# bxh1/VIDO-SLAM

Hardware: AMD Instinct MI355X
Metric: frames/sec end-to-end (flow+depth+track+local-BA) at 640x480; BA iters/sec (higher is better)
Workload: dtype f32

## Files before the change

include/vido_c.h:

```cpp
#ifndef VIDO_C_H
#define VIDO_C_H
#include <stdint.h>
#include <stddef.h>
#ifdef __cplusplus
extern "C" {
#endif

#define VIDO_OK              0
#define VIDO_E_INVALID      -1
#define VIDO_E_NO_DEVICE    -2
#define VIDO_E_HIP          -3
#define VIDO_E_CAPACITY     -4
#define VIDO_E_NOMEM        -5

#define VIDO_MAX_LEVELS 16

typedef struct vido_ctx vido_ctx;

typedef struct vido_keypoint { float x, y, size, angle, response; int32_t octave; } vido_keypoint;

typedef struct vido_config {
    int32_t device;
    int32_t width, height;
    int32_t max_batch;
// ... 159 lines not shown

typedef struct vido_ba_dynamic {
    int32_t n_H, n_dyn, n_tern, n_smooth;
    double* H_T;
    double* dyn_xyz;
    const int32_t* dyn_cam; const double* dyn_meas;
    const int32_t* tern_prev; const int32_t* tern_cur; const int32_t* tern_H;
    const int32_t* sm_i; const int32_t* sm_j;
    double info_dyn, info_tern, info_smooth, huber_dyn, huber_tern, huber_smooth;
} vido_ba_dynamic;
int vido_ba_optimize_dynamic(vido_ctx* ctx, vido_ba_problem* prob, vido_ba_dynamic* dyn, vido_ba_result* result,
                             vido_allreduce_fn allreduce, void* user);

int vido_correlation(vido_ctx* ctx, const float* first, const float* second, int B, int C, int H, int W, int stride,
                     float* out, int on_device);
int vido_det_order(vido_ctx* ctx, const float* scores, const long long* labels, const int* n_det, float confidence, int cap, long long* order, long long* labels_out, long long* n_live);
int vido_det_order_n(vido_ctx* ctx, const float* scores, const long long* labels, const int* n_det, float confidence, int cap, long long* order, long long* labels_out, long long* n_live,
                     int32_t* n_live32);
int vido_roi_levels(vido_ctx* ctx, const float* boxes, int n, float k_min, float k_max, int* out);
int vido_mask_logit_select(vido_ctx* ctx, const float* feat, const float* w, const float* b, const long long* labels, float* out, int n, int c, int hw, int classes);
int vido_mask_logit_select_n(vido_ctx* ctx, const float* feat, const float* w, const float* b, const long long* labels, float* out, int n, int c, int hw, int classes, const int32_t* n_live);
int vido_bias_act(vido_ctx* ctx, float* x, const float* bias, int N, int C, int H, int W, float slope);
int vido_bias_unary(vido_ctx* ctx, float* x, const float* bias, int N, int C, int H, int W, int kind);
int vido_upcat_reflect(vido_ctx* ctx, const float* x, const float* skip, int C1, int C2, int h, int w, float* out);
int vido_minmax_norm_u16(vido_ctx* ctx, const float* d, const float* mm, int64_t n, int32_t* out);
int vido_bias_res_act(vido_ctx* ctx, float* x, const float* bias, const float* res, int N, int C, int H, int W, float slope);
int vido_area_feed(vido_ctx* ctx, const uint8_t* bgr, int H, int W, float* out, int OH, int OW, float div);
int vido_backwarp(vido_ctx* ctx, const float* x, const float* flow, int B, int C, int H, int W, float* out);
int vido_deconv4s2_depthwise(vido_ctx* ctx, const float* x, const float* weight, int B, int C, int H, int W, float input_slope, float* out);

int vido_conv1x1_supported(int cin, int cout, int hw);
int vido_conv1x1_layout(int cin, int cout, int hw);
int vido_conv1x1_set_arith(int arith);
int vido_conv1x1_range_flag(vido_ctx* ctx, int reset);
int vido_range_latch(vido_ctx* ctx, unsigned* dst);
int vido_conv1x1_bias_act(vido_ctx* ctx, const float* x, const float* w_packed, const float* bias, const float* residual, float* y, int cin, int cout, int hw, float slope);
int vido_deconv2x2_supported(int n, int cin, int cout, int h, int w);
int vido_deconv2x2_bias_act(vido_ctx* ctx, const float* x, const float* w_packed, const float* bias, float* y, int n, int cin, int cout, int h, int w, float slope);
int vido_deconv2x2_bias_act_n(vido_ctx* ctx, const float* x, const float* w_packed, const float* bias, float* y, int n, int cin, int cout, int h, int w, float slope, const int32_t* n_live);
int vido_conv1x1_bias_up2_act(vido_ctx* ctx, const float* x, const float* w_packed, const float* bias, const float* residual_half, float* y, int cin, int cout, int h, int w, float slope);

int vido_conv_kxk_c2(vido_ctx* ctx, const float* x, const float* w, const float* bias, const float* residual, float* y, int cin, int k, int h, int w_);
int vido_conv1x1_skinny(vido_ctx* ctx, const float* x, const float* w_packed, const float* bias, const float* residual, float* y, int cin, int cout, long long hw, float slope);
int vido_stem7x7s2_pool(vido_ctx* ctx, const float* x, const float* w_packed, const float* bias, float* y, int h, int w);

int vido_conv_direct_supported(int cin, int cout, int h, int w, int kh, int kw, int sh, int sw, int ph, int pw);
long long vido_conv_direct_packed_floats(int cin, int cout, int kh, int kw);
int vido_conv_direct_pack(const float* w, int cin, int cout, int kh, int kw, float* w_packed);
int vido_conv_direct_bias_act(vido_ctx* ctx, const float* x, const float* w_packed, const float* bias, float* y, int n, int cin, int cout, int h, int w,
                              int kh, int kw, int sh, int sw, int ph, int pw, float slope);

int vido_wino3x3_supported(int cin, int cout, int h, int w);
int vido_wino3x3_fills_chip(int n, int cout, int h, int w, int min_wgs);
long long vido_wino3x3_packed_floats(int cin, int cout);
int vido_wino3x3_pack(const float* w, int cin, int cout, float* u_packed);
int vido_wino3x3_bias_act(vido_ctx* ctx, const float* x, const float* u_packed, const float* bias, float* y, int n, int cin, int cout, int h, int w, float slope);
int vido_wino3x3_form(int n, int cin, int cout, int h, int w);
int vido_fc_h_splitk(int rows, int k, int outs);
int vido_fc_h(vido_ctx* ctx, const float* x, const void* w_packed, const float* bias, float* part, float* y, int rows, int k, int outs, float slope);
int vido_conv3x3_h_supported(int n, int cin, int cout, int h, int w);
int vido_conv3x3_h_workgroups(int n, int cout, int h, int w);
int vido_conv3x3_h_bias_act(vido_ctx* ctx, const float* x, const void* w_packed, const float* bias, float* y, int n, int cin, int cout, int h, int w, float slope);
int vido_conv3x3_h_bias_act_n(vido_ctx* ctx, const float* x, const void* w_packed, const float* bias, float* y, int n, int cin, int cout, int h, int w, float slope, const int32_t* n_live);
int vido_conv3x3_h_live_form(int n, int cout, int h, int w, int live, int* channels, int* block_rows);
int vido_mask_head_coarse(void);
int vido_conv3x3_h_bias_act_form(vido_ctx* ctx, const float* x, const void* w_packed, const float* bias, float* y, int n, int cin, int cout, int h, int w, float slope, int rpw, int cg);
long long vido_wino3x3_packed_floats_form(int cin, int cout, int form);
int vido_wino3x3_pack_form(const float* w, int cin, int cout, int form, float* u_packed);
int vido_wino3x3_bias_act_form(vido_ctx* ctx, const float* x, const float* u_packed, const float* bias, float* y, int n, int cin, int cout, int h, int w, float slope, int form);
int vido_gconv3x3_supported(int H, int W, int cpg_in, int cpg_out);
int64_t vido_gconv3x3_packed_size(int groups, int cpg_in, int cpg_out);
int vido_gconv3x3_bias_act(vido_ctx* ctx, const float* x, const float* in_bias, const float* w_packed, const float* bias, float* y, int groups, int cpg_in, int cpg_out, int H, int W, float slope);
int vido_gconv3x3_s2_supported(int H, int W, int cpg_in, int cpg_out);
int vido_gconv3x3_s2_bias_act(vido_ctx* ctx, const float* x, const float* w_packed, const float* bias, float* y, int groups, int cpg_in, int cpg_out, int H, int W, float slope);
int vido_lfn_reg_front(vido_ctx* ctx, const float* im1, const float* im2, const float* flow, const float* mean, float scale, int B, int C, int H, int W, float* out, int out_channels);
int vido_lfn_reg_tail(vido_ctx* ctx, const float* dist, const float* flow, const float* wx, const float* bx, const float* wy, const float* by, int B, int K, int H, int W, float* out);
int vido_roi_align(vido_ctx* ctx, const float* feat, int B, int C, int H, int W, const float* rois, int n_rois,
                   float spatial_scale, int pooled_h, int pooled_w, int sampling_ratio, float* out, int on_device);
int vido_nms(vido_ctx* ctx, const float* boxes_xyxy, const float* scores, int n, float thresh, int32_t* keep_out,
             int32_t* n_keep, int on_device);
int vido_nms_grouped(vido_ctx* ctx, const float* boxes_xyxy, const float* scores, const int32_t* groups, int n, float thresh,
                     int32_t* keep_out, int32_t* n_keep, int on_device);
int vido_nms_segments(vido_ctx* ctx, const float* boxes_xyxy, const int32_t* groups, const int32_t* seg_off, const int32_t* seg_n, int n_seg, int max_n, int total,
                      float thresh, int32_t* keep_out, int32_t* n_keep);
int vido_roi_align_fpn(vido_ctx* ctx, const float* const feat[4], const int H[4], const int W[4], const float scale[4], int C, const float* boxes, const int32_t* level,
                       int n, int pooled_h, int pooled_w, int sampling_ratio, float* out);
int vido_nchw_to_nhwc(vido_ctx* ctx, const float* src, int B, int C, int H, int W, float* dst);
int vido_roi_align_fpn_nhwc(vido_ctx* ctx, const float* const feat[4], const int H[4], const int W[4], const float scale[4], int C, const float* boxes, const int32_t* level,
                            int n, int pooled_h, int pooled_w, int sampling_ratio, float* out);
int vido_roi_align_fpn_nhwc_n(vido_ctx* ctx, const float* const feat[4], const int H[4], const int W[4], const float scale[4], int C, const float* boxes, const int32_t* level,
                              int n, int pooled_h, int pooled_w, int sampling_ratio, float* out, const int32_t* n_live);
int vido_bawin_create(vido_ctx* ctx, int cap_frames, int cap_features);
int vido_bawin_push_frame(vido_ctx* ctx, int frame, int n, const double* meas, const float* xyz, const int32_t* asso);
int vido_bawin_set_labels(vido_ctx* ctx, int n, const int32_t* quads);
int vido_bawin_solve(vido_ctx* ctx, int start, int N, vido_ba_problem* prob, vido_ba_result* res, int32_t* n_obs_out, int32_t* n_pt_out);
int vido_bawin_read_points(vido_ctx* ctx, int frame, int n, float* xyz_out);
int vido_rpn_select(vido_ctx* ctx, int n_levels, const float* const* logits, const float* const* deltas, const int* h, const int* w, const int* stride, const float* cell_anchors,
                    int A, int K, int img_w, int img_h, float* boxes_out, float* scores_out, int32_t* n_out);
int vido_rpn_merge(vido_ctx* ctx, const float* boxes, const float* scores, const int32_t* keep, const int32_t* cnt, int n_levels, int K, int post_nms_top_n, int n_final,
                   float* out_boxes, float* out_scores, int32_t* n_valid);
int vido_det_class_sort(vido_ctx* ctx, const float* prob, const float* deltas, const float* proposals, const float* objectness, int N, int nc, float thresh, const float weights[4],
                        int img_w, int img_h, float* seg_boxes, int32_t* order, int32_t* seg_n);
int vido_det_select(vido_ctx* ctx, const float* prob, const float* seg_boxes, const int32_t* order, const int32_t* keep, const int32_t* cnt, int N, int nc, int detections_per_img, int cap,
                    int32_t* scratch, float* out_boxes, float* out_scores, int64_t* out_labels, int32_t* n_det);
int vido_mask_label_image(vido_ctx* ctx, const float* masks, const float* boxes, const int64_t* labels, int n, int M, int padding, float thresh, int H, int W, uint8_t* out);
// ... 81 lines not shown
```

vido-slam_amd/csrc/conv1x1.hip:

```cpp
#include "common.hpp"
#include <atomic>

namespace {
typedef float f32x16 __attribute__((ext_vector_type(16)));
typedef float f32x4 __attribute__((ext_vector_type(4)));
typedef float f32x2 __attribute__((ext_vector_type(2)));

#define C1_TM 128
#define C1_TN 128

struct C1Args { const float* x; const float* wp; const float* bias; const float* res; float* y; int M, N, K, mt, total, nchunk; float slope; unsigned xbytes, wbytes; int W; unsigned* range_flag; int hwimg, c4; const int* n_live; };

template <int RES, int KC>
__global__ __launch_bounds__(256) void k_conv1x1(C1Args A)
{
    constexpr int NG = KC / 8;
    constexpr int A_BUF = 4 * NG * 256, B_BUF = KC * C1_TN;
    constexpr int NPW = KC / 4;
    extern __shared__ __attribute__((aligned(16))) float c1_lds[];
    float* Al = c1_lds; float* Bl = c1_lds + 2 * A_BUF;
    const int tid = threadIdx.x, lane = tid & 63, w = __builtin_amdgcn_readfirstlane(tid >> 6), wm = w & 1, wn = w >> 1;
    const int per = gridDim.x >> 3, item = (blockIdx.x & 7) * per + (blockIdx.x >> 3);
    if (item >= A.total) return;
    const int nt = item / A.mt, mtile = item - nt * A.mt, n0 = nt * C1_TN, m0 = mtile * C1_TM;
// ... 413 lines not shown
    } else {
        float* X = (float*)L;
        if (g == 0) { ep_load(0, E0); ep_load(1, E1); } else { ep_load(2, E0); ep_load(3, E1); }
        __builtin_amdgcn_s_barrier();
        auto put = [&](int which, const f32x16& v0, const f32x16& v1) {
            float* Pw = X + (((which * 4 + w) * 2) * 16) * 64 + lane;
#pragma unroll
            for (int r = 0; r < 16; r++) { Pw[r * 64] = v0[r]; Pw[(16 + r) * 64] = v1[r]; }
        };
        if (g == 1) put(0, acc[0], acc[1]); else put(1, acc[2], acc[3]);
        __syncthreads();
        const float* Pr = X + (((g * 4 + w) * 2) * 16) * 64 + lane;
        if (g == 0) { ep_store(0, acc[0], Pr, E0); ep_store(1, acc[1], Pr + 16 * 64, E1); }
        else { ep_store(2, acc[2], Pr, E0); ep_store(3, acc[3], Pr + 16 * 64, E1); }
    }
}
}

extern "C" {

int vido_conv1x1_supported(int cin, int cout, int hw)
{
    return cin >= 32 && cin % 32 == 0 && cout >= C1_TM && cout % C1_TM == 0 && hw >= C1_TN && 4ll * cin * hw < (1ll << 32) && 4ll * cin * cout < (1ll << 32);
}

static std::atomic<int>& c1_arith()
{
    static std::atomic<int> v{[] { const char* e = getenv("VIDO_CONV1X1_ARITH");
                                   return (e && !strcmp(e, "f32")) || (!e && getenv("VIDO_CONV1X1_TN")) ? 1 : (e && (!strcmp(e, "bf16x3") || !strcmp(e, "bf16"))) ? 2 : 0; }()};
    return v;
}

int vido_conv1x1_set_arith(int arith) { return c1_arith().exchange(arith == 1 ? 1 : arith == 2 ? 2 : 0); }

int vido_conv1x1_range_flag(vido_ctx* ctx, int reset)
{
    if (!ctx || !ctx->c1_range_flag) return 0;
    return reset ? (int)__atomic_exchange_n(ctx->c1_range_flag, 0u, __ATOMIC_ACQ_REL) : (int)__atomic_load_n(ctx->c1_range_flag, __ATOMIC_ACQUIRE);
}

int vido_conv1x1_layout(int cin, int cout, int hw)
{
    { const int ar = c1_arith().load(std::memory_order_relaxed); if (ar != 1) return ar == 2 ? 2 : 3; }
    static const int force = [] { const char* e = getenv("VIDO_CONV1X1_TN"); return e ? atoi(e) : 128; }();
    if (force == 128 || cin % 64 != 0) return 0;
    if (force == 112) return 1;
    const long long mt = cout / C1_TM, t128 = mt * ((hw + 127) / 128), t112 = mt * ((hw + C2_TN - 1) / C2_TN);
    const long long c128 = ((t128 + 255) / 256) * 128, c112 = ((t112 + 255) / 256) * C2_TN;
    return c112 < c128 ? 1 : 0;
}

static int c1_launch(vido_ctx* ctx, const float* x, const float* w_packed, const float* bias, const float* residual, int res_mode, float* y, int cin, int cout, int hw, int w, float slope,
                     int hwimg = 0, int c4 = 0, const int32_t* n_live = nullptr)
{
    if (!ctx) return VIDO_E_INVALID;
    if (!x || !w_packed || !y || x == y || !vido_conv1x1_supported(cin, cout, hw) || slope < 0.f || slope > 1.f || (((uintptr_t)x | (uintptr_t)y | (uintptr_t)residual | (uintptr_t)n_live) & 3) || ((uintptr_t)w_packed & 15))
        return vido_set_error(ctx, VIDO_E_INVALID, "conv1x1: no kernel for %d -> %d channels at %d positions (or a pointer is misaligned, or slope outside [0, 1])", cin, cout, hw);
    HIP_TRY(ctx, hipSetDevice(ctx->device));
    hipStream_t st = ctx->has_ext_stream ? ctx->ext_stream : ctx->stream;
    const int rm = res_mode == 3 ? 3 : (residual ? res_mode : 0);
    const int layout = vido_conv1x1_layout(cin, cout, hw);
    if ((hwimg || rm == 3) && layout != 3) return vido_set_error(ctx, VIDO_E_INVALID, "conv1x1: the batch / transposed-convolution forms exist in the split-fp16 arithmetic only");
    if (layout >= 2) {
        const int np = layout == 3 ? 2 : 3;
        const int mt = cout / C1_TM, ntl = (hw + C1_TN - 1) / C1_TN, total = mt * ntl;
        C1Args A{x, w_packed, bias, residual, y, cout, hw, cin, mt, total, cin / 16, slope, (unsigned)(4ll * cin * hw), (unsigned)(2ll * np * cin * cout), w, ctx->c1_range_flag, hwimg, c4, n_live};
// ... 88 lines not shown
```

vido-slam_amd/nets/fuse.py:

```python
import os
import torch
import torch.nn as nn
import torch.nn.functional as F


def _fold(conv, bn, eps):
    scale = bn.weight * (bn.running_var + eps).rsqrt()
    w = conv.weight * scale.reshape(-1, 1, 1, 1)
    b = bn.bias - bn.running_mean * scale
    if conv.bias is not None:
        b = b + conv.bias * scale
    return w.detach().contiguous(), b.detach().contiguous()


def _eps(bn):
    return float(getattr(bn, "eps", 0.0))


def fold_batchnorm(net, ops):
    from .maskrcnn import _Bottleneck, _Stem
    from .monodepth2 import _Basic, ResnetEncoder18, DepthDecoder
    n = 0
    for m in net.modules():
        if isinstance(m, _Bottleneck):
            m._w1, m._b1 = _fold(m.conv1, m.bn1, _eps(m.bn1)); m._w2, m._b2 = _fold(m.conv2, m.bn2, _eps(m.bn2)); m._w3, m._b3 = _fold(m.conv3, m.bn3, _eps(m.bn3)); n += 3
            if m.downsample is not None:
                m._wd, m._bd = _fold(m.downsample[0], m.downsample[1], _eps(m.downsample[1])); n += 1
            m._ep = ops.bias_res_act_
            c2 = m.conv2; m._w2p = None; m._ops = ops
            if c2.groups > 1 and tuple(c2.stride) == (1, 1) and tuple(c2.padding) == (1, 1) and tuple(c2.dilation) == (1, 1) and not os.environ.get("VIDO_NO_GCONV"):
                from .ops import pack_gconv3x3
                m._w2p = pack_gconv3x3(m._w2, c2.groups)
            elif (c2.groups > 1 and tuple(c2.stride) == (2, 2) and tuple(c2.padding) == (1, 1) and tuple(c2.dilation) == (1, 1) and ((c2.out_channels // c2.groups) % 32 == 0 or (c2.out_channels // c2.groups) in (8, 16))
                  and not os.environ.get("VIDO_NO_GCONV") and not os.environ.get("VIDO_NO_GCONV_S2")):
                from .ops import pack_gconv3x3
                m._w2p = pack_gconv3x3(m._w2, c2.groups)
            m._w1p = m._w3p = m._wdp = None; m._c1x1_min_tiles = 0
            mode = os.environ.get("VIDO_CONV1X1", "all")
            if not os.environ.get("VIDO_NO_CONV1X1") and hasattr(ops, "conv1x1_bias_act"):
                from .ops import PackedConv1x1
                m._w3p = PackedConv1x1.make(m._w3)
                if mode == "all":
                    if tuple(m.conv1.stride) == (1, 1): m._w1p = PackedConv1x1.make(m._w1)
                    if m.downsample is not None and tuple(m.downsample[0].stride) in ((1, 1), (2, 2)): m._wdp = PackedConv1x1.make(m._wd)
        elif isinstance(m, _Stem):
            m._w1, m._b1 = _fold(m.conv1, m.bn1, _eps(m.bn1)); m._ep = ops.bias_res_act_; n += 1
        elif isinstance(m, _Basic):
            m._w1, m._b1 = _fold(m.conv1, m.bn1, m.bn1.eps); m._w2, m._b2 = _fold(m.conv2, m.bn2, m.bn2.eps); n += 2
            if m.downsample is not None:
                m._wd, m._bd = _fold(m.downsample[0], m.downsample[1], m.downsample[1].eps); n += 1
            m._ep = ops.bias_res_act_
        elif isinstance(m, DepthDecoder):
            m._ops = ops if hasattr(ops, "upcat_reflect") and not os.environ.get("VIDO_NO_DEPTH_FUSED") else None
        elif isinstance(m, ResnetEncoder18):
            e = m.encoder
            w, b = _fold(e.conv1, e.bn1, e.bn1.eps)
            m._w1, m._b1 = w, b; m._ep = ops.bias_res_act_; n += 1
    return n


class Graphed:

    def __init__(self, fn, example_inputs, warmup=2):
        self.fn = fn
        self.static_in = [x.clone() for x in example_inputs]
# ... 19 lines not shown
```

vido-slam_amd/nets/maskrcnn.py:

```python
import math
import os
from collections import OrderedDict
from dataclasses import dataclass
import numpy as np
import torch
import torch.nn as nn
import torch.nn.functional as F


@dataclass
class MaskRCNNConfig:
    blocks: tuple = (3, 4, 23, 3)
    groups: int = 32
    width_per_group: int = 8
    stride_in_1x1: bool = False
    stem_out: int = 64
    res2_out: int = 256
    fpn_out: int = 256
    anchor_sizes: tuple = (32, 64, 128, 256, 512)
    aspect_ratios: tuple = (0.5, 1.0, 2.0)
    anchor_strides: tuple = (4, 8, 16, 32, 64)
    pre_nms_top_n: int = 1000
    post_nms_top_n: int = 1000
    fpn_post_nms_top_n: int = 1000
# ... 7 lines not shown
    score_thresh: float = 0.05
    nms: float = 0.5
    detections_per_img: int = 100
    bbox_reg_weights: tuple = (10.0, 10.0, 5.0, 5.0)
    mask_resolution: int = 14
    mask_layers: tuple = (256, 256, 256, 256)


class FrozenBatchNorm2d(nn.Module):
    def __init__(self, n):
        super().__init__()
        for name, v in (("weight", torch.ones(n)), ("bias", torch.zeros(n)), ("running_mean", torch.zeros(n)), ("running_var", torch.ones(n))):
            self.register_buffer(name, v)

    def forward(self, x):
        scale = self.weight * self.running_var.rsqrt()
        bias = self.bias - self.running_mean * scale
        return x * scale.reshape(1, -1, 1, 1) + bias.reshape(1, -1, 1, 1)


class _Bottleneck(nn.Module):
    def __init__(self, cin, mid, cout, groups, stride_in_1x1, stride):
        super().__init__()
        self.downsample = None
        if cin != cout:
            self.downsample = nn.Sequential(nn.Conv2d(cin, cout, 1, stride, bias=False), FrozenBatchNorm2d(cout))
        s1, s3 = (stride, 1) if stride_in_1x1 else (1, stride)
        self.conv1 = nn.Conv2d(cin, mid, 1, s1, bias=False); self.bn1 = FrozenBatchNorm2d(mid)
        self.conv2 = nn.Conv2d(mid, mid, 3, s3, 1, bias=False, groups=groups); self.bn2 = FrozenBatchNorm2d(mid)
        self.conv3 = nn.Conv2d(mid, cout, 1, bias=False); self.bn3 = FrozenBatchNorm2d(cout)

    _ep = None
    _w2p = None
    _w1p = _w3p = _wdp = None; _c1x1_min_tiles = 0

    def forward(self, x):
        if self._ep is not None and x.is_cuda:
            ep = self._ep; c1, c2 = self.conv1, self.conv2; ops = self._ops
            b1x = x.shape[0] == 1 and not getattr(ops, "_range_safe", 0)
            hw_in = x.shape[2] * x.shape[3]
            b1_done = False
            from .ops import conv1x1_fills_chip as fills
            if self._w1p is not None and b1x and ops.conv1x1_supported(x.shape[1], self._w1.shape[0], hw_in) and fills(self._w1.shape[0], hw_in):
                y = ops.conv1x1_bias_act(x.contiguous(), self._w1p, self._b1, None, 0.0); b1_done = True
            else:
                y = F.conv2d(x, self._w1, None, c1.stride)
            if (self._w2p is not None and tuple(c2.stride) == (2, 2)):
                if b1_done and y.shape[0] == 1 and self._ops.gconv3x3_s2_supported(y.shape[2], y.shape[3], c2.in_channels // c2.groups, c2.out_channels // c2.groups):
                    y = self._ops.gconv3x3_s2_bias_act(y, self._w2p, self._b2, c2.groups, 0.0)
                else:
                    y = ep(F.conv2d(y if b1_done else ep(y, self._b1, None, 0.0), self._w2, None, c2.stride, c2.padding, c2.dilation, c2.groups), self._b2, None, 0.0)
            elif self._w2p is not None and y.shape[0] == 1 and self._ops.gconv3x3_supported(y.shape[2], y.shape[3], c2.in_channels // c2.groups, c2.out_channels // c2.groups):
                y = self._ops.gconv3x3_bias_act(y, self._w2p, self._b2, c2.groups, 0.0, in_bias=None if b1_done else self._b1)
            else:
                y = ep(F.conv2d(y if b1_done else ep(y, self._b1, None, 0.0), self._w2, None, c2.stride, c2.padding, c2.dilation, c2.groups), self._b2, None, 0.0)
            if self.downsample is None:
                sc = x
            elif self._wdp is not None and b1x and tuple(self.downsample[0].stride) == (1, 1) and ops.conv1x1_supported(x.shape[1], self._wd.shape[0], hw_in) and fills(self._wd.shape[0], hw_in):
                sc = ops.conv1x1_bias_act(x.contiguous(), self._wdp, self._bd, None, 1.0)
            elif (self._wdp is not None and b1x and tuple(self.downsample[0].stride) == (2, 2) and ops.conv1x1_supported(x.shape[1], self._wd.shape[0], ((x.shape[2] + 1) // 2) * ((x.shape[3] + 1) // 2))
                  and fills(self._wd.shape[0], ((x.shape[2] + 1) // 2) * ((x.shape[3] + 1) // 2))):
                sc = ops.conv1x1_bias_act(x[:, :, ::2, ::2].contiguous(), self._wdp, self._bd, None, 1.0)
            else:
                sc = ep(F.conv2d(x, self._wd, None, self.downsample[0].stride), self._bd, None, 1.0)
            if (self._w3p is not None and b1x and y.shape[0] == 1 and ops.conv1x1_supported(y.shape[1], self._w3.shape[0], y.shape[2] * y.shape[3])
                    and (fills(self._w3.shape[0], y.shape[2] * y.shape[3]) or self._c1x1_min_tiles < 0)):
                return ops.conv1x1_bias_act(y.contiguous(), self._w3p, self._b3, sc, 0.0)
            return ep(F.conv2d(y, self._w3), self._b3, sc.contiguous(), 0.0)
        y = F.relu(self.bn1(self.conv1(x)))
        y = F.relu(self.bn2(self.conv2(y)))
        y = self.bn3(self.conv3(y))
        return F.relu(y + (x if self.downsample is None else self.downsample(x)))


class _Stem(nn.Module):
    def __init__(self, cout):
        super().__init__()
        self.conv1 = nn.Conv2d(3, cout, 7, 2, 3, bias=False); self.bn1 = FrozenBatchNorm2d(cout)

    _ep = None

    def forward(self, x):
        if self._ep is not None and x.is_cuda:
            ops = getattr(self._ep, "__self__", None)
            if x.shape[0] == 1 and hasattr(ops, "stem7x7s2_pool_conv") and not os.environ.get("VIDO_NO_STEM_FUSED"):
                y = ops.stem7x7s2_pool_conv(self, self._w1, self._b1, x)
# ... 650 lines not shown
```

vido-slam_amd/nets/ops.py:

```python
import contextlib
import ctypes as C
import os
import torch

_WINO_MIN_WGS = int(os.environ.get("VIDO_WINO_MIN_WGS", "0"))
_CONV3X3_H_MIN_WGS = 0 if os.environ.get("VIDO_CONV3X3_H") == "0" else int(os.environ.get("VIDO_CONV3X3_H_MIN_WGS", "128"))
_CONVDIRECT_SET = os.environ.get("VIDO_CONVDIRECT_SET", "novalu")


def correlation_torch_reference(first, second, stride):
    a, b = first[:, :, ::stride, ::stride], second[:, :, ::stride, ::stride]
    pad = torch.nn.functional.pad(b, (3, 3, 3, 3))
    H, W = a.shape[2], a.shape[3]
    return torch.stack([(a * pad[:, :, p:p + H, o:o + W]).mean(1) for p in range(7) for o in range(7)], 1)


class HipOps:

    _range_safe = 0

    def __init__(self, ctx):
        self.ctx = ctx

    @property
    def range_safe_active(self):
        return self._range_safe > 0

    @staticmethod
    def _live_ptr(n_live):
        if n_live is None:
            return None
        assert n_live.is_cuda and n_live.dtype == torch.int32 and n_live.numel() == 1, "n_live: a one-element int32 device tensor"
        return C.c_void_p(n_live.data_ptr())

    def _adopt_stream(self):
        st = torch.cuda.current_stream().cuda_stream
        self.ctx._check(self.ctx.lib.vido_set_stream(self.ctx.h, C.c_void_p(st), 1))

    def correlation(self, first, second, stride):
        if not first.is_cuda:
# ... 106 lines not shown
        self.ctx._check(self.ctx.lib.vido_area_feed(self.ctx.h, C.c_void_p(bgr.data_ptr()), bgr.shape[0], bgr.shape[1], C.c_void_p(out.data_ptr()), int(feed[0]), int(feed[1]), C.c_float(div)))
        return out

    def backwarp(self, x, flow):
        assert x.is_cuda and x.dtype == torch.float32 and flow.dtype == torch.float32 and x.shape[0] == flow.shape[0] and x.shape[2:] == flow.shape[2:] and flow.shape[1] == 2
        x = x.contiguous(); flow = flow.contiguous()
        out = torch.empty_like(x)
        self._adopt_stream()
        self.ctx._check(self.ctx.lib.vido_backwarp(self.ctx.h, C.c_void_p(x.data_ptr()), C.c_void_p(flow.data_ptr()), x.shape[0], x.shape[1], x.shape[2], x.shape[3], C.c_void_p(out.data_ptr())))
        return out

    def deconv4s2_depthwise(self, x, weight, input_slope=1.0):
        x = x.contiguous(); B, Cc, H, W = x.shape
        assert weight.shape == (Cc, 1, 4, 4) and weight.is_contiguous()
        out = torch.empty((B, Cc, 2 * H, 2 * W), device=x.device, dtype=torch.float32)
        self._adopt_stream()
        self.ctx._check(self.ctx.lib.vido_deconv4s2_depthwise(self.ctx.h, C.c_void_p(x.data_ptr()), C.c_void_p(weight.data_ptr()), B, Cc, H, W, C.c_float(input_slope), C.c_void_p(out.data_ptr())))
        return out

    def gconv3x3_supported(self, H, W, cpg_in, cpg_out):
        return bool(self.ctx.lib.vido_gconv3x3_supported(int(H), int(W), int(cpg_in), int(cpg_out)))

    def gconv3x3_bias_act(self, x, w_packed, bias, groups, slope=0.0, in_bias=None):
        assert x.is_cuda and x.is_contiguous() and x.dtype == torch.float32 and x.shape[0] == 1
        _, Cin, H, W = x.shape
        cpg_in = Cin // groups; cpg_out = bias.numel() // groups
        out = torch.empty((1, bias.numel(), H, W), device=x.device, dtype=torch.float32)
        self.gconv_flops = getattr(self, "gconv_flops", 0.0) + 2.0 * bias.numel() * cpg_in * 9 * H * W
        self._adopt_stream()
        self.ctx._check(self.ctx.lib.vido_gconv3x3_bias_act(self.ctx.h, C.c_void_p(x.data_ptr()), C.c_void_p(in_bias.data_ptr()) if in_bias is not None else None,
                                                            C.c_void_p(w_packed.data_ptr()), C.c_void_p(bias.data_ptr()), C.c_void_p(out.data_ptr()),
                                                            int(groups), cpg_in, cpg_out, H, W, C.c_float(slope)))
        return out

    def gconv3x3_s2_supported(self, H, W, cpg_in, cpg_out):
        return bool(self.ctx.lib.vido_gconv3x3_s2_supported(int(H), int(W), int(cpg_in), int(cpg_out)))

    def gconv3x3_s2_bias_act(self, x, w_packed, bias, groups, slope=0.0):
        assert x.is_cuda and x.is_contiguous() and x.dtype == torch.float32 and x.shape[0] == 1
        _, Cin, H, W = x.shape
        cpg_in = Cin // groups; cpg_out = bias.numel() // groups
        out = torch.empty((1, bias.numel(), (H + 1) // 2, W // 2), device=x.device, dtype=torch.float32)
        self.gconv_flops = getattr(self, "gconv_flops", 0.0) + 2.0 * bias.numel() * cpg_in * 9 * out.shape[2] * out.shape[3]
        self._adopt_stream()
        self.ctx._check(self.ctx.lib.vido_gconv3x3_s2_bias_act(self.ctx.h, C.c_void_p(x.data_ptr()), C.c_void_p(w_packed.data_ptr()), C.c_void_p(bias.data_ptr()), C.c_void_p(out.data_ptr()),
                                                               int(groups), cpg_in, cpg_out, H, W, C.c_float(slope)))
        return out

    def conv1x1_supported(self, cin, cout, hw):
        return bool(self.ctx.lib.vido_conv1x1_supported(int(cin), int(cout), int(hw)))

    def conv1x1_set_arith(self, arith):
        return int(self.ctx.lib.vido_conv1x1_set_arith(int(arith)))

    def range_latch(self, dst):
        assert dst.dtype == torch.int32 and dst.numel() >= 1 and dst.is_contiguous() and (dst.is_cuda or dst.is_pinned()), "range_latch: an int32 word on the device or pinned"
        self._adopt_stream()
        self.ctx._check(self.ctx.lib.vido_range_latch(self.ctx.h, C.c_void_p(dst.data_ptr())))
        return dst

    def conv1x1_range_flag(self, reset=True):
        return int(self.ctx.lib.vido_conv1x1_range_flag(self.ctx.h, int(bool(reset))))

    def conv1x1_layout(self, cin, cout, hw):
        return int(self.ctx.lib.vido_conv1x1_layout(int(cin), int(cout), int(hw)))

# ... 749 lines not shown
        key = (int(layout), str(device))
        if key not in self._p:
            p = pack_conv1x1(self.w, layout)
            assert p is not None, "conv1x1: layout %d does not take %d -> %d channels" % (layout, self.cin, self.cout)
            self._p[key] = p.to(device)
        return self._p[key]


def pack_conv1x1_skinny(w):
    cout, cin = int(w.shape[0]), int(w.shape[1])
    cop = (cout + 31) // 32 * 32
    wz = w.detach().reshape(cout, cin).new_zeros((cop, cin)); wz[:cout] = w.detach().reshape(cout, cin)
    return wz.reshape(cop // 32, 32, cin // 2, 2).permute(0, 2, 3, 1).contiguous().reshape(cop // 32, cin // 2, 64)


def pack_stem7x7(w):
    assert tuple(w.shape) == (64, 3, 7, 7)
    wz = w.detach().new_zeros((64, 3, 8, 7)); wz[:, :, :7] = w.detach()
    return wz.reshape(2, 32, 3, 4, 2, 7).permute(0, 2, 5, 3, 4, 1).contiguous().reshape(2, 84, 64)


def pack_gconv3x3(w, groups):
    cout, cpg_in = int(w.shape[0]), int(w.shape[1])
    cpg_out = cout // groups
    if tuple(w.shape[2:]) != (3, 3) or cpg_in % 8 or not (cpg_out % 32 == 0 or cpg_out in (8, 16)):
        return None
    w9 = w.detach().reshape(groups, cpg_out, cpg_in // 8, 8, 9)
    if cpg_out % 32 == 0:
        return w9.reshape(groups, cpg_out // 32, 32, cpg_in // 8, 8, 9).permute(0, 1, 3, 5, 4, 2).contiguous()
    pad = w9.new_zeros((groups, 16, cpg_in // 8, 8, 9)); pad[:, :cpg_out] = w9
    return pad.permute(0, 2, 4, 3, 1).contiguous()


def pack_conv_direct(w):
    import numpy as np
    from ..host import load_library
    lib = load_library()
    lib.vido_conv_direct_packed_floats.restype = C.c_longlong
    cout, cin, kh, kw = (int(v) for v in w.shape)
    wh = np.ascontiguousarray(w.detach().to("cpu", torch.float32).numpy())
    n = int(lib.vido_conv_direct_packed_floats(cin, cout, kh, kw))
    if n <= 0:
        raise RuntimeError("vido_conv_direct_pack: no kernel for %d x %d taps" % (kh, kw))
    out = np.empty(n, np.float32)
    rc = lib.vido_conv_direct_pack(C.c_void_p(wh.ctypes.data), cin, cout, kh, kw, C.c_void_p(out.ctypes.data))
    if rc != 0:
        raise RuntimeError("vido_conv_direct_pack: %d" % rc)
    return torch.from_numpy(out)


def pack_wino3x3(w, form=0):
    import numpy as np
    from ..host import load_library
    lib = load_library()
    lib.vido_wino3x3_packed_floats_form.restype = C.c_longlong
    cout, cin = int(w.shape[0]), int(w.shape[1])
    assert tuple(w.shape[2:]) == (3, 3) and form in (0, 1, 2)
    wh = np.ascontiguousarray(w.detach().to("cpu", torch.float32).numpy())
    n = int(lib.vido_wino3x3_packed_floats_form(cin, cout, int(form)))
    out = np.empty(n, np.float32)
    rc = lib.vido_wino3x3_pack_form(C.c_void_p(wh.ctypes.data), cin, cout, int(form), C.c_void_p(out.ctypes.data))
    if rc != 0:
        raise RuntimeError("vido_wino3x3_pack_form: %d" % rc)
    kc = 8 if (((cout + 63) // 64) * 64 - cout) < 32 and form == 0 else 4
    cop = ((cout + 63) // 64) * 64 if kc == 8 else ((cout + 31) // 32) * 32
    cip = ((cin + kc - 1) // kc) * kc
# ... 2 lines not shown
```

Measured before the change: 132.1.

## Add split-fp16 MFMA grouped 3x3 conv kernel and route eligible layers to it

Adds a grouped 3x3 stride-1 convolution kernel for 32 or 64 channels per group. Weights and activations are each split into high and low fp16 halves and multiplied with three 32x32x16 f16 MFMA ops per step, which approximates f32 accuracy. Weights are staged into LDS through buffer loads, and input bands are double-buffered in LDS. Python dispatch sends eligible ResNeXt conv2 layers to the new kernel when there is no input bias, range-safe mode is off and conv1x1 arith is not mode 1. The aim is to replace the existing f32 grouped conv with tensor-core work, at the cost of a range check on activations that must stay below 65504 and a small precision risk.

```diff
diff --git a/include/vido_c.h b/include/vido_c.h
--- a/include/vido_c.h
+++ b/include/vido_c.h
@@ -215,6 +215,7 @@
 int vido_conv1x1_supported(int cin, int cout, int hw);
 int vido_conv1x1_layout(int cin, int cout, int hw);
 int vido_conv1x1_set_arith(int arith);
+int vido_conv1x1_get_arith(void);
 int vido_conv1x1_range_flag(vido_ctx* ctx, int reset);
 int vido_range_latch(vido_ctx* ctx, unsigned* dst);
 int vido_conv1x1_bias_act(vido_ctx* ctx, const float* x, const float* w_packed, const float* bias, const float* residual, float* y, int cin, int cout, int hw, float slope);
@@ -254,6 +255,8 @@
 int vido_gconv3x3_supported(int H, int W, int cpg_in, int cpg_out);
 int64_t vido_gconv3x3_packed_size(int groups, int cpg_in, int cpg_out);
 int vido_gconv3x3_bias_act(vido_ctx* ctx, const float* x, const float* in_bias, const float* w_packed, const float* bias, float* y, int groups, int cpg_in, int cpg_out, int H, int W, float slope);
+int vido_gconv3x3_h_supported(int H, int W, int cpg_in, int cpg_out);
+int vido_gconv3x3_h_bias_act(vido_ctx* ctx, const float* x, const void* w_packed, const float* bias, float* y, int groups, int cpg_in, int cpg_out, int H, int W, float slope);
 int vido_gconv3x3_s2_supported(int H, int W, int cpg_in, int cpg_out);
 int vido_gconv3x3_s2_bias_act(vido_ctx* ctx, const float* x, const float* w_packed, const float* bias, float* y, int groups, int cpg_in, int cpg_out, int H, int W, float slope);
 int vido_lfn_reg_front(vido_ctx* ctx, const float* im1, const float* im2, const float* flow, const float* mean, float scale, int B, int C, int H, int W, float* out, int out_channels);
diff --git a/vido-slam_amd/csrc/conv1x1.hip b/vido-slam_amd/csrc/conv1x1.hip
--- a/vido-slam_amd/csrc/conv1x1.hip
+++ b/vido-slam_amd/csrc/conv1x1.hip
@@ -469,6 +469,7 @@
 }
 
 int vido_conv1x1_set_arith(int arith) { return c1_arith().exchange(arith == 1 ? 1 : arith == 2 ? 2 : 0); }
+int vido_conv1x1_get_arith(void) { return c1_arith().load(std::memory_order_relaxed); }
 
 int vido_conv1x1_range_flag(vido_ctx* ctx, int reset)
 {
diff --git a/vido-slam_amd/csrc/gconvh.hip b/vido-slam_amd/csrc/gconvh.hip
--- /dev/null
+++ b/vido-slam_amd/csrc/gconvh.hip
@@ -0,0 +1,189 @@
+#include "common.hpp"
+
+namespace {
+typedef float f32x16 __attribute__((ext_vector_type(16)));
+typedef _Float16 f16x8 __attribute__((ext_vector_type(8)));
+
+#define GH_OOB 0x40000000u
+#define GH_CUS 256
+
+struct GhArgs { const float* x; const void* wp; const float* bias; float* y; unsigned* range_flag; int H, W, gx, total, CL, BPX, BP, nunits; float slope; unsigned xbytes, wbytes, m_wp, m_bpx; };
+
+template <int CPG> struct GhForm {
+    static constexpr int NCG = CPG / 8, NKS = CPG / 16, NCOB = CPG / 32;
+    static constexpr int MAXU = CPG == 32 ? 5 : 7;
+    static_assert(MAXU <= 7, "the kernel's unit arrays hold seven");
+    static constexpr int MAXBP = MAXU * 256 / NCG;
+    static constexpr int WB = NKS * 18 * 1024;
+};
+
+template <int CPG>
+__global__ __launch_bounds__(256) void k_gconv3x3_h(GhArgs A)
+{
+    typedef GhForm<CPG> F;
+    constexpr int NCG = F::NCG, NKS = F::NKS, NCOB = F::NCOB, MAXU = F::MAXU, WB = F::WB;
+    extern __shared__ __attribute__((aligned(16))) char gh_lds[];
+    char* const WL = gh_lds;
+    char* const PH = gh_lds + WB;
+    const int tid = threadIdx.x, lane = tid & 63, wv = __builtin_amdgcn_readfirstlane(tid >> 6);
+    const int H = A.H, W = A.W, Wp = W + 2, npos = H * Wp, BPX = A.BPX, BP = A.BP;
+    const unsigned HW = (unsigned)H * (unsigned)W, PLANE = (unsigned)(NCG * BP) * 16u;
+    const int per = gridDim.x >> 3, item = (blockIdx.x & 7) * per + (blockIdx.x >> 3);
+    if (item >= A.total) return;
+    const int gc = item / A.gx, chunk = item - gc * A.gx, g = gc / NCOB, cob = gc - g * NCOB;
+    const int qc = chunk * A.CL, qn = min(A.CL, npos - qc), nrounds = (qn + 127) >> 7;
+
+    {
+        const __amdgpu_buffer_rsrc_t wr = __builtin_amdgcn_make_buffer_rsrc((void*)A.wp, 0, A.wbytes, 0x00020000);
+#pragma unroll
+        for (int i = 0; i < NKS * 18 / 4; i++) {
+            const int piece = wv + 4 * i;
+            __builtin_amdgcn_raw_ptr_buffer_load_lds(wr, (__attribute__((address_space(3))) void*)(WL + piece * 1024), 16, 16u * (unsigned)lane, (unsigned)gc * (unsigned)WB + 1024u * (unsigned)piece, 0, 0);
+        }
+    }
+    const __amdgpu_buffer_rsrc_t xr = __builtin_amdgcn_make_buffer_rsrc((void*)A.x, 0, A.xbytes, 0x00020000);
+    const unsigned xbase = 4u * (unsigned)(g * CPG) * HW;
+    int ui[7]; unsigned ucg[7];
+#pragma unroll
+    for (int j = 0; j < MAXU; j++) { const unsigned u = (unsigned)(tid + 256 * j), cg = __umulhi(u, A.m_bpx); ucg[j] = u < (unsigned)A.nunits ? cg : 0xffffffffu; ui[j] = (int)(u - cg * (unsigned)BPX); }
+    float pre[7][8];
+    auto load_band = [&](int q0) {
+#pragma unroll
+        for (int j = 0; j < MAXU; j++) {
+            const unsigned f = (unsigned)(q0 + ui[j]), yr = __umulhi(f, A.m_wp), xc = f - yr * (unsigned)Wp;
+            const bool ok = ucg[j] != 0xffffffffu && yr >= 1u && yr <= (unsigned)H && xc >= 1u && xc <= (unsigned)W;
+            const unsigned vo = ok ? 4u * (ucg[j] * 8u * HW + (yr - 1u) * (unsigned)W + (xc - 1u)) : GH_OOB;
+#pragma unroll
+            for (int e = 0; e < 8; e++) pre[j][e] = __builtin_bit_cast(float, __builtin_amdgcn_raw_buffer_load_b32(xr, vo, xbase + 4u * (unsigned)e * HW, 0));
+        }
+    };
+    float xmax = 0.f;
+    auto convert = [&]() {
+#pragma unroll
+        for (int j = 0; j < MAXU; j++) {
+            f16x8 h8, l8;
+#pragma unroll
+            for (int e = 0; e < 8; e++) {
+                const float v = pre[j][e];
+                const _Float16 h = (_Float16)v;
+                const float r = __builtin_fmaf((float)h, -2048.f, v * 2048.f);
+                h8[e] = h; l8[e] = (_Float16)r;
+                xmax = __builtin_elementwise_maximum(xmax, __builtin_fabsf(v));
+            }
+            if (ucg[j] != 0xffffffffu) {
+                const unsigned o = (ucg[j] * (unsigned)BP + (unsigned)ui[j]) * 16u;
+                *(f16x8*)(PH + o) = h8; *(f16x8*)(PH + PLANE + o) = l8;
+            }
+        }
+    };
+
+    const int co_base = g * CPG + cob * 32;
+    const float* wsc = (const float*)((const char*)A.wp + A.wbytes);
+    float bv[16], sv[16];
+#pragma unroll
+    for (int r = 0; r < 16; r++) { const int co = co_base + 8 * (r >> 2) + 4 * (lane >> 5) + (r & 3); bv[r] = A.bias[co]; sv[r] = wsc[co]; }
+
+    load_band(qc);
+    convert();
+    asm volatile("s_waitcnt vmcnt(0)" ::: "memory");
+    typedef const __attribute__((address_space(3))) f16x8* lds_h8;
+    for (int rd = 0; rd < nrounds; rd++) {
+        __syncthreads();
+        if (rd + 1 < nrounds) load_band(qc + 128 * (rd + 1));
+        const int qt = qc + 128 * rd + 32 * wv;
+        if (128 * rd + 32 * wv < qn) {
+            f32x16 acc, acl;
+#pragma unroll
+            for (int r = 0; r < 16; r++) { acc[r] = 0.f; acl[r] = 0.f; }
+            const unsigned a_lane = 16u * (unsigned)lane;
+            const unsigned b_lane = ((unsigned)(lane >> 5) * (unsigned)BP + (unsigned)(32 * wv + (lane & 31))) * 16u;
+            f16x8 ah[3], al[3], bh[3], bl[3];
+            auto ld = [&](int s) {
+                const int tap = s / NKS, ks = s - tap * NKS;
+                const char* ap = WL + ((ks * 9 + tap) * 2) * 1024 + a_lane;
+                const char* bp = PH + b_lane + (unsigned)((tap / 3) * Wp + tap % 3) * 16u + (unsigned)(2 * ks * BP) * 16u;
+                ah[s % 3] = *(lds_h8)ap; al[s % 3] = *(lds_h8)(ap + 1024);
+                bh[s % 3] = *(lds_h8)bp; bl[s % 3] = *(lds_h8)(bp + PLANE);
+            };
+            ld(0); ld(1);
+#pragma unroll
+            for (int s = 0; s < 9 * NKS; s++) {
+                if (s + 2 < 9 * NKS) ld(s + 2);
+                __builtin_amdgcn_sched_barrier(0);
+                acl = __builtin_amdgcn_mfma_f32_32x32x16_f16(ah[s % 3], bl[s % 3], acl, 0, 0, 0);
+                acc = __builtin_amdgcn_mfma_f32_32x32x16_f16(ah[s % 3], bh[s % 3], acc, 0, 0, 0);
+                acl = __builtin_amdgcn_mfma_f32_32x32x16_f16(al[s % 3], bh[s % 3], acl, 0, 0, 0);
+                __builtin_amdgcn_sched_barrier(0);
+            }
+            const int q = qt + (lane & 31), yy = (int)__umulhi((unsigned)q, A.m_wp), xx = q - yy * Wp;
+            if (q < npos && xx < W) {
+                float* yo = A.y + (size_t)co_base * HW + (size_t)yy * W + xx;
+#pragma unroll
+                for (int r = 0; r < 16; r++) {
+                    const int co = 8 * (r >> 2) + 4 * (lane >> 5) + (r & 3);
+                    const float v = (acc[r] + acl[r] * 0x1p-11f) * sv[r] + bv[r];
+                    yo[(size_t)co * HW] = fmaxf(v, v * A.slope);
+                }
+            }
+        }
+        if (rd + 1 < nrounds) {
+            __syncthreads();
+            convert();
+        }
+    }
+    if (!(xmax < 65504.f) && A.range_flag) atomicOr(A.range_flag, 1u);
+}
+
+struct GhPlan { int gx, CL, BPX, BP, nunits; size_t lds; };
+static GhPlan gh_plan(int groups, int H, int W, int cpg_in, int cpg_out)
+{
+    GhPlan p{};
+    if (H < 1 || W < 1 || cpg_in != cpg_out || (cpg_in != 32 && cpg_in != 64)) return p;
+    const int ncg = cpg_in / 8, ncob = cpg_in / 32, maxbp = cpg_in == 32 ? GhForm<32>::MAXBP : GhForm<64>::MAXBP;
+    const long long Wp = W + 2, npos = (long long)H * Wp, bpx = 130 + 2 * Wp;
+    if (bpx > maxbp || (npos + 2 * bpx + 256) * Wp >= (1ll << 32)) return p;
+    p.BPX = (int)bpx; p.BP = (p.BPX + 15) & ~15; p.nunits = p.BPX * ncg;
+    p.lds = (size_t)(cpg_in / 16) * 18 * 1024 + (size_t)2 * ncg * p.BP * 16;
+    static const int force = [] { const char* e = getenv("VIDO_GCONV_H_ITEMS"); return e ? atoi(e) : 0; }();
+    const int per_cu = std::max(1, (int)(160 * 1024 / p.lds)), target = force > 0 ? force : GH_CUS * std::min(per_cu, 2);
+    const int ntile = (int)((npos + 31) / 32), gcs = std::max(groups, 1) * ncob;
+    int gx = std::min(std::max((target + gcs / 2) / gcs, 1), ntile);
+    p.CL = ((ntile + gx - 1) / gx) * 32;
+    p.gx = (int)((npos + p.CL - 1) / p.CL);
+    return p;
+}
+}
+
+extern "C" {
+
+int vido_gconv3x3_h_supported(int H, int W, int cpg_in, int cpg_out)
+{
+    return gh_plan(1, H, W, cpg_in, cpg_out).gx != 0;
+}
+
+int vido_gconv3x3_h_bias_act(vido_ctx* ctx, const float* x, const void* w_packed, const float* bias, float* y, int groups, int cpg_in, int cpg_out, int H, int W, float slope)
+{
+    if (!ctx) return VIDO_E_INVALID;
+    if (!x || !w_packed || !bias || !y || (const void*)x == (const void*)y || groups < 1 || groups > 65535 || !(slope >= 0.f && slope <= 1.f) || (((uintptr_t)x | (uintptr_t)y) & 3) || ((uintptr_t)w_packed & 15))
+        return vido_set_error(ctx, VIDO_E_INVALID, "gconv3x3_h: bad arguments");
+    const GhPlan p = gh_plan(groups, H, W, cpg_in, cpg_out);
+    const long long xb = 4ll * groups * cpg_in * H * W, wb = 36ll * groups * cpg_out * cpg_in;
+    if (!p.gx || xb >= (1ll << 30) || wb >= (1ll << 31)) return vido_set_error(ctx, VIDO_E_INVALID, "gconv3x3_h: no kernel for %d -> %d channels per group at %d x %d", cpg_in, cpg_out, H, W);
+    HIP_TRY(ctx, hipSetDevice(ctx->device));
+    static bool attr[64] = {};
+    if (!attr[ctx->device & 63]) {
+        HIP_TRY(ctx, hipFuncSetAttribute((const void*)k_gconv3x3_h<32>, hipFuncAttributeMaxDynamicSharedMemorySize, 160 * 1024));
+        HIP_TRY(ctx, hipFuncSetAttribute((const void*)k_gconv3x3_h<64>, hipFuncAttributeMaxDynamicSharedMemorySize, 160 * 1024));
+        attr[ctx->device & 63] = true;
+    }
+    hipStream_t st = ctx->has_ext_stream ? ctx->ext_stream : ctx->stream;
+    auto magic = [](unsigned d) { return (unsigned)((0x100000000ull + d - 1) / d); };
+    const int total = p.gx * groups * (cpg_out / 32);
+    GhArgs A{x, w_packed, bias, y, ctx->c1_range_flag, H, W, p.gx, total, p.CL, p.BPX, p.BP, p.nunits, slope, (unsigned)xb, (unsigned)wb, magic((unsigned)(W + 2)), magic((unsigned)p.BPX)};
+    const dim3 grid(8 * ((total + 7) / 8)), blk(256);
+    if (cpg_in == 32) hipLaunchKernelGGL(k_gconv3x3_h<32>, grid, blk, p.lds, st, A); else hipLaunchKernelGGL(k_gconv3x3_h<64>, grid, blk, p.lds, st, A);
+    HIP_TRY(ctx, hipGetLastError());
+    return VIDO_OK;
+}
+
+}
diff --git a/vido-slam_amd/nets/fuse.py b/vido-slam_amd/nets/fuse.py
--- a/vido-slam_amd/nets/fuse.py
+++ b/vido-slam_amd/nets/fuse.py
@@ -27,10 +27,11 @@
             if m.downsample is not None:
                 m._wd, m._bd = _fold(m.downsample[0], m.downsample[1], _eps(m.downsample[1])); n += 1
             m._ep = ops.bias_res_act_
-            c2 = m.conv2; m._w2p = None; m._ops = ops
+            c2 = m.conv2; m._w2p = None; m._w2ph = None; m._ops = ops
             if c2.groups > 1 and tuple(c2.stride) == (1, 1) and tuple(c2.padding) == (1, 1) and tuple(c2.dilation) == (1, 1) and not os.environ.get("VIDO_NO_GCONV"):
-                from .ops import pack_gconv3x3
+                from .ops import pack_gconv3x3, pack_gconv3x3_h
                 m._w2p = pack_gconv3x3(m._w2, c2.groups)
+                m._w2ph = pack_gconv3x3_h(m._w2, c2.groups) if m._w2p is not None else None
             elif (c2.groups > 1 and tuple(c2.stride) == (2, 2) and tuple(c2.padding) == (1, 1) and tuple(c2.dilation) == (1, 1) and ((c2.out_channels // c2.groups) % 32 == 0 or (c2.out_channels // c2.groups) in (8, 16))
                   and not os.environ.get("VIDO_NO_GCONV") and not os.environ.get("VIDO_NO_GCONV_S2")):
                 from .ops import pack_gconv3x3
diff --git a/vido-slam_amd/nets/maskrcnn.py b/vido-slam_amd/nets/maskrcnn.py
--- a/vido-slam_amd/nets/maskrcnn.py
+++ b/vido-slam_amd/nets/maskrcnn.py
@@ -63,6 +63,7 @@
 
     _ep = None
     _w2p = None
+    _w2ph = None
     _w1p = _w3p = _wdp = None; _c1x1_min_tiles = 0
 
     def forward(self, x):
@@ -82,7 +83,7 @@
                 else:
                     y = ep(F.conv2d(y if b1_done else ep(y, self._b1, None, 0.0), self._w2, None, c2.stride, c2.padding, c2.dilation, c2.groups), self._b2, None, 0.0)
             elif self._w2p is not None and y.shape[0] == 1 and self._ops.gconv3x3_supported(y.shape[2], y.shape[3], c2.in_channels // c2.groups, c2.out_channels // c2.groups):
-                y = self._ops.gconv3x3_bias_act(y, self._w2p, self._b2, c2.groups, 0.0, in_bias=None if b1_done else self._b1)
+                y = self._ops.gconv3x3_conv(y, self._w2p, self._w2ph, self._b2, c2.groups, 0.0, in_bias=None if b1_done else self._b1)
             else:
                 y = ep(F.conv2d(y if b1_done else ep(y, self._b1, None, 0.0), self._w2, None, c2.stride, c2.padding, c2.dilation, c2.groups), self._b2, None, 0.0)
             if self.downsample is None:
diff --git a/vido-slam_amd/nets/ops.py b/vido-slam_amd/nets/ops.py
--- a/vido-slam_amd/nets/ops.py
+++ b/vido-slam_amd/nets/ops.py
@@ -6,6 +6,7 @@
 _WINO_MIN_WGS = int(os.environ.get("VIDO_WINO_MIN_WGS", "0"))
 _CONV3X3_H_MIN_WGS = 0 if os.environ.get("VIDO_CONV3X3_H") == "0" else int(os.environ.get("VIDO_CONV3X3_H_MIN_WGS", "128"))
 _CONVDIRECT_SET = os.environ.get("VIDO_CONVDIRECT_SET", "novalu")
+_GCONV_H = os.environ.get("VIDO_GCONV_H", "1") != "0"
 
 
 def correlation_torch_reference(first, second, stride):
@@ -178,6 +179,28 @@
                                                             C.c_void_p(w_packed.data_ptr()), C.c_void_p(bias.data_ptr()), C.c_void_p(out.data_ptr()),
                                                             int(groups), cpg_in, cpg_out, H, W, C.c_float(slope)))
         return out
+
+    def gconv3x3_h_supported(self, H, W, cpg_in, cpg_out):
+        return bool(self.ctx.lib.vido_gconv3x3_h_supported(int(H), int(W), int(cpg_in), int(cpg_out)))
+
+    def gconv3x3_h_bias_act(self, x, w_packed, bias, groups, slope=0.0):
+        assert x.is_cuda and x.is_contiguous() and x.dtype == torch.float32 and x.shape[0] == 1
+        _, Cin, H, W = x.shape
+        cpg = Cin // groups
+        assert bias.numel() == Cin and w_packed.dtype == torch.int16 and w_packed.numel() == 2 * Cin * (cpg * 9 + 1), "gconv3x3_h: weight not packed by pack_gconv3x3_h for this layer"
+        out = torch.empty((1, Cin, H, W), device=x.device, dtype=torch.float32)
+        self.gconv_flops = getattr(self, "gconv_flops", 0.0) + 2.0 * Cin * cpg * 9 * H * W
+        self._adopt_stream()
+        self.ctx._check(self.ctx.lib.vido_gconv3x3_h_bias_act(self.ctx.h, C.c_void_p(x.data_ptr()), C.c_void_p(w_packed.data_ptr()), C.c_void_p(bias.data_ptr()), C.c_void_p(out.data_ptr()),
+                                                              int(groups), cpg, cpg, H, W, C.c_float(slope)))
+        return out
+
+    def gconv3x3_conv(self, x, w_packed, w_packed_h, bias, groups, slope=0.0, in_bias=None):
+        cpg = x.shape[1] // groups
+        if (_GCONV_H and w_packed_h is not None and in_bias is None and not self._range_safe and int(self.ctx.lib.vido_conv1x1_get_arith()) != 1
+                and bias.numel() == x.shape[1] and self.gconv3x3_h_supported(x.shape[2], x.shape[3], cpg, cpg)):
+            return self.gconv3x3_h_bias_act(x, w_packed_h, bias, groups, slope)
+        return self.gconv3x3_bias_act(x, w_packed, bias, groups, slope, in_bias=in_bias)
 
     def gconv3x3_s2_supported(self, H, W, cpg_in, cpg_out):
         return bool(self.ctx.lib.vido_gconv3x3_s2_supported(int(H), int(W), int(cpg_in), int(cpg_out)))
@@ -993,6 +1016,16 @@
     return pad.permute(0, 2, 4, 3, 1).contiguous()
 
 
+def pack_gconv3x3_h(w, groups):
+    cout, cpg = int(w.shape[0]), int(w.shape[1])
+    if w.dim() != 4 or tuple(w.shape[2:]) != (3, 3) or groups < 1 or cout != groups * cpg or cpg not in (32, 64):
+        return None
+    h, l, inv = split_f16x2(w.detach().reshape(cout, cpg * 9))
+    planes = torch.stack([h, l], 0).view(torch.int16).reshape(2, groups, cpg // 32, 32, cpg // 16, 2, 8, 9)
+    planes = planes.permute(1, 2, 4, 7, 0, 5, 3, 6).contiguous().reshape(-1)
+    return torch.cat([planes, inv.contiguous().view(torch.int16).reshape(-1)])
+
+
 def pack_conv_direct(w):
     import numpy as np
     from ..host import load_library
```

Result: faster. 136.1 (median of 6 runs) (+3.0%).
